# DanielQ-51/cudapathtracer

Measured on AMD Instinct MI355X. Metric: Mray/s, higher is better.
Workload: dtype f32; 1 GPU; cornell_1920x1080_1024spp_depth8_mis; spp=1024, max_depth=8, integrator=UNIDIRECTIONAL (MIS), variant=megakernel, seed=103033, triangles=36, bvh_nodes=31

## Files before the change

cudapathtracer_amd/csrc/pt_device.h:

```cpp
#pragma once
#include <hip/hip_runtime.h>
#include <stdint.h>

#define PT_DEV __device__ __forceinline__

namespace pt {

constexpr float kEps = 0.00001f;
constexpr float kRayEps = 0.001f;
constexpr float kPi = 3.141592f;

struct V3 { float x, y, z; };

PT_DEV V3 v3(float x, float y, float z) { return V3{x, y, z}; }
PT_DEV V3 v3(float a) { return V3{a, a, a}; }
PT_DEV V3 operator+(V3 a, V3 b) { return V3{a.x + b.x, a.y + b.y, a.z + b.z}; }
PT_DEV V3 operator-(V3 a, V3 b) { return V3{a.x - b.x, a.y - b.y, a.z - b.z}; }
PT_DEV V3 operator*(V3 a, float t) { return V3{a.x * t, a.y * t, a.z * t}; }
PT_DEV V3 operator*(float t, V3 a) { return V3{a.x * t, a.y * t, a.z * t}; }
PT_DEV V3 operator*(V3 a, V3 b) { return V3{a.x * b.x, a.y * b.y, a.z * b.z}; }
PT_DEV V3 operator/(V3 a, float t) { return V3{a.x / t, a.y / t, a.z / t}; }
PT_DEV V3 operator/(V3 a, V3 b) { return V3{a.x / b.x, a.y / b.y, a.z / b.z}; }
PT_DEV V3 operator-(V3 a) { return V3{-a.x, -a.y, -a.z}; }

PT_DEV float dot(V3 a, V3 b) { return __builtin_fmaf(a.z, b.z, __builtin_fmaf(a.y, b.y, a.x * b.x)); }
PT_DEV V3 cross(V3 a, V3 b) {
    return V3{__builtin_fmaf(a.y, b.z, -(a.z * b.y)), __builtin_fmaf(a.z, b.x, -(a.x * b.z)), __builtin_fmaf(a.x, b.y, -(a.y * b.x))};
}
PT_DEV float fminf_(float a, float b) { return __builtin_fminf(a, b); }
PT_DEV float fmaxf_(float a, float b) { return __builtin_fmaxf(a, b); }
#ifndef PT_FAST_RCP
#define PT_FAST_RCP 1
#endif
#ifndef PT_RCP_UNIFORM
#define PT_RCP_UNIFORM 1
#endif
PT_DEV float rcp_exact(float a) {
#if PT_FAST_RCP && PT_RCP_UNIFORM
    const float m = __builtin_fabsf(a);
    const float r0 = __builtin_amdgcn_rcpf(a);
    float r = __builtin_fmaf(r0, __builtin_fmaf(-a, r0, 1.0f), r0);
    const bool inRange = m >= 1e-12f && m <= 1.0e30f;
    if (__builtin_expect(__builtin_amdgcn_ballot_w64(!inRange) != 0ull, 0)) r = inRange ? r : 1.0f / a;
    return r;
#else
#if PT_FAST_RCP
    const float m = __builtin_fabsf(a);
    if (m >= 1e-12f && m <= 1.0e30f) {
        const float r0 = __builtin_amdgcn_rcpf(a);
        return __builtin_fmaf(r0, __builtin_fmaf(-a, r0, 1.0f), r0);
    }
#endif
    return 1.0f / a;
#endif
}
PT_DEV float rsqrt_(float x) { return rcp_exact(__builtin_sqrtf(x)); }
PT_DEV V3 normalize(V3 v) { float il = rsqrt_(dot(v, v)); return V3{v.x * il, v.y * il, v.z * il}; }
PT_DEV float length(V3 v) { return __builtin_sqrtf(dot(v, v)); }
PT_DEV float clampf(float x, float lo, float hi) { return x < lo ? lo : (x > hi ? hi : x); }

PT_DEV void sincos_(float x, float& s, float& c) {
    float k = __builtin_rintf(x * 0.636619772f);
    float r = __builtin_fmaf(k, -1.5703125f, x);
    r = __builtin_fmaf(k, -4.837512969970703125e-4f, r);
    r = __builtin_fmaf(k, -7.54978995489188216e-8f, r);
    int q = (int)k;
    float r2 = r * r;
    float ps = __builtin_fmaf(r2, -1.9515295891e-4f, 8.3321608736e-3f);
    ps = __builtin_fmaf(ps, r2, -1.6666654611e-1f);
    float sn = __builtin_fmaf(r * r2, ps, r);
    float pc = __builtin_fmaf(r2, 2.443315711809948e-5f, -1.388731625493765e-3f);
    pc = __builtin_fmaf(pc, r2, 4.166664568298827e-2f);
    float cs = __builtin_fmaf(r2 * r2, pc, __builtin_fmaf(r2, -0.5f, 1.0f));
    bool swap = q & 1;
    float a = swap ? cs : sn, b = swap ? sn : cs;
    s = (q & 2) ? -a : a;
    c = ((q + 1) & 2) ? -b : b;
}

PT_DEV float exp_(float x) {
    if (x != x) return x;
    if (x > 88.5f) return __builtin_inff();
    if (x < -87.0f) return 0.0f;
    float n = __builtin_rintf(x * 1.44269504f);
    float r = __builtin_fmaf(n, -0.693359375f, x);
    r = __builtin_fmaf(n, 2.12194440e-4f, r);
    float p = __builtin_fmaf(r, 1.9875691500e-4f, 1.3981999507e-3f);
    p = __builtin_fmaf(p, r, 8.3334519073e-3f);
// ... 108 lines not shown
```

cudapathtracer_amd/csrc/pt_megakernel.h:

```cpp
#pragma once
#include "pt_path.h"
#include "pt_params.h"

namespace pt {

PT_DEV void wave_add_total(unsigned long long* totals, int k, uint32_t v) {
    unsigned long long s = v;
    for (int off = 32; off > 0; off >>= 1) s += __shfl_down(s, off, 64);
    if ((threadIdx.x & 63) == 0 && s) atomicAdd(&totals[k], s);
}

extern __shared__ __attribute__((aligned(16))) unsigned char pt_smem[];

PT_DEV SceneCache stage_scene_cache(const DeviceScene& S, int cacheNodes, int cacheTris, int attrOff = 0, int nA = 0, int nM = 0, int nL = 0) {
    typedef __attribute__((address_space(3))) f4v lds_f4;
    lds_f4* dstN = (lds_f4*)pt_smem;
    lds_f4* dstT = dstN + cacheNodes * 4;
    const f4v* srcN = reinterpret_cast<const f4v*>(S.nodes);
    const f4v* srcT = reinterpret_cast<const f4v*>(S.tris);
    for (int i = threadIdx.x; i < cacheNodes * 4; i += blockDim.x) dstN[i] = srcN[i];
    for (int i = threadIdx.x; i < cacheTris * 3; i += blockDim.x) dstT[i] = srcT[i];
    if (attrOff > 0) {
        lds_f4* dA = (lds_f4*)(pt_smem + attrOff);
        lds_f4* dM = dA + nA * 5;
// ... 62 lines not shown
                    } else if (tmo == 0ull || now - t0 > 4ull * tmo) {
                        atomicOr((unsigned*)&q[3], 2u);
                        break;
                    }
                }
            }
            __builtin_amdgcn_s_sleep(64);
        }
    }
    return __builtin_amdgcn_readfirstlane(item);
}
PT_DEV void queue_push(int* q, int mask, int item, int lane) {
    if (lane == 0) {
        const unsigned pos = atomicAdd((unsigned*)&q[1], 1u);
        unsigned long long* slot = queue_slot(q, mask, pos);
        const unsigned long long t0 = wall_clock64();
        while ((unsigned)PT_QLOAD(slot) != pos) {
            if ((PT_QLOAD(&q[3]) & 6) != 0) return;
            if (wall_clock64() - t0 > queue_timeout(q)) { atomicOr((unsigned*)&q[3], 4u); return; }
            __builtin_amdgcn_s_sleep(4);
        }
        PT_QSTORE(slot, ((unsigned long long)(unsigned)item << 32) | (unsigned long long)(pos + 1u));
    }
}
PT_DEV uint32_t state_load(const uint32_t* p, bool shared) { return shared ? PT_QLOAD(p) : *p; }
PT_DEV void state_store(uint32_t* p, uint32_t v, bool shared) { if (shared) PT_QSTORE(p, v); else *p = v; }

template <int INTEG, bool COUNT, bool DEFER, bool ONCHIP, int STACKN, bool CULL = false, bool REFILL = false, bool FLAT = false, bool SIMPLE = false, int FLATW = 1, int TREE = 0, bool LEAN = false,
          bool MOMENTS = false>
PT_DEV void megakernel_body(const KParams& P, const MomentsK& M = MomentsK{nullptr, nullptr, 0, 0.0f}) {
    static_assert(!MOMENTS || !COUNT, "the fused moments render has no counting form");
    constexpr bool NOLEAF = SIMPLE || LEAN || (DEFER && FLAT);
    constexpr bool LTRI = DEFER && FLAT && SIMPLE;
#ifndef PT_TRISEL_SIMPLE4
#define PT_TRISEL_SIMPLE4 1
#endif
    constexpr bool TRISEL = ((PT_TRISEL_LEAN != 0 && LEAN && !SIMPLE) || (PT_TRISEL_SIMPLE4 != 0 && SIMPLE && STACKN == kStackLds)) && !ONCHIP && !COUNT;
    const int wave = threadIdx.x >> 6, lane = threadIdx.x & 63, nW = blockDim.x >> 6;
    DeviceScene S = P.S;
    constexpr bool ATTRLDS = ONCHIP && kAttrCacheBytes > 0;
    constexpr int kMedBytes = SIMPLE ? 0 : kMediumMax * 64;
    const int attrOff = ATTRLDS ? P.cacheNodes * 64 + P.cacheTris * 48 + nW * (STACKN * 256 + kMedBytes) : 0;
    DeviceScene Sstage = S;
#ifdef PT_EXPERIMENTAL
    constexpr bool WIDE = TREE == 1, COMPACT = TREE == 2;
    if (WIDE) Sstage.nodes = reinterpret_cast<const PNode*>(P.wnodes);
    if (COMPACT) Sstage.nodes = reinterpret_cast<const PNode*>(P.qnodes);
#else
    static_assert(TREE == 0, "the wide / compact trees are -DPT_EXPERIMENTAL builds (pt_trace_experimental.h)");
#endif
    const SceneCache SC = stage_scene_cache(Sstage, P.cacheNodes, P.cacheTris, attrOff, P.cacheAttrs, P.cacheMats, P.cacheLights);
    if constexpr (ATTRLDS) {
        typedef __attribute__((address_space(3))) const PAttr lds_attr;
        typedef __attribute__((address_space(3))) const PMat lds_mat;
        typedef __attribute__((address_space(3))) const PLight lds_light;
        lds_attr* a = (lds_attr*)(pt_smem + attrOff);
        lds_mat* m = (lds_mat*)(pt_smem + attrOff + P.cacheAttrs * 80);
        lds_light* l = (lds_light*)(pt_smem + attrOff + P.cacheAttrs * 80 + P.cacheMats * 96);
        S.attrs = (const PAttr*)a; S.mats = (const PMat*)m; S.lights = (const PLight*)l;
    }
    int vb = blockIdx.x;
#ifdef PT_EXPERIMENTAL
    if (P.xcdBands) {
        const int nB = gridDim.x, q = nB >> 3, r = nB & 7, x = vb & 7;
        vb = x * q + (x < r ? x : r) + (vb >> 3);
    }
// ... 176 lines not shown
                const Compact K{P.qnodes, reinterpret_cast<const f4v*>(P.leafBox), P.mids};
                trace_resume_q<STACKN>(S, SC, K, st, rs, ps.o, ps.d, (nBusy * P.refillKeep) >> 4, thr, h, Keep{P.nodeKeep, P.triKeep});
                PT_STAMP(1);
                continue;
            }
            if constexpr (WIDE) {
                trace_resume_w4<STACKN>(S, SC, P.wnodes, st, rs, ps.o, ps.d, (nBusy * P.refillKeep) >> 4, thr, h, c, Keep{P.nodeKeep, P.triKeep});
                if (!(rs.flags & kRayBusy) && (rs.flags & kRayTie)) {
                    SceneCache none; none.nodes = nullptr; none.nNodes = 0; none.tris = nullptr; none.nTris = 0;
                    trace_closest_plain<false, STACKN, false, false>(S, none, ps.o, ps.d, 999999.0f, st, h, c);
                    rs.flags &= ~kRayTie;
                }
                PT_STAMP(1);
                continue;
            }
#endif
#if !defined(PT_EXPERIMENTAL)
            trace_resume<COUNT, STACKN, ONCHIP, NOLEAF, TRISEL>(S, SC, st, rs, ps.o, ps.d, (nBusy * P.refillKeep) >> 4, thr, h, c, Keep{P.nodeKeep, P.triKeep});
#elif PT_SPEC == 2
            if (P.spec) trace_resume_spec<COUNT, STACKN, ONCHIP, NOLEAF>(S, SC, st, rs, ps.o, ps.d, (nBusy * P.refillKeep) >> 4, thr, h, c, Keep{P.nodeKeep, P.triKeep}, P.spec == 2);
            else trace_resume<COUNT, STACKN, ONCHIP, NOLEAF, TRISEL>(S, SC, st, rs, ps.o, ps.d, (nBusy * P.refillKeep) >> 4, thr, h, c, Keep{P.nodeKeep, P.triKeep});
#elif PT_SPEC == 1
            trace_resume_spec<COUNT, STACKN, ONCHIP, NOLEAF>(S, SC, st, rs, ps.o, ps.d, (nBusy * P.refillKeep) >> 4, thr, h, c, Keep{P.nodeKeep, P.triKeep}, P.spec == 2);
#else
            trace_resume<COUNT, STACKN, ONCHIP, NOLEAF, TRISEL>(S, SC, st, rs, ps.o, ps.d, (nBusy * P.refillKeep) >> 4, thr, h, c, Keep{P.nodeKeep, P.triKeep});
#endif
            PT_STAMP(1);
            continue;
        }
#ifdef PT_STAMPS
        occ[0] += 64; occ[1] += __builtin_popcountll(__ballot((ps.flags & kInPath) != 0 || (samplesLeft > 0 && !stopStarting)));
#endif
        const uint32_t flagsIn = ps.flags;
        if (DEFER) apply_pending<NOLEAF>(ps, thr, acc);
        if constexpr (MOMENTS && DEFER) landed_by_apply(flagsIn);
        if (ps.flags & kInPath) {
            bool done = path_bounce<INTEG, COUNT, DEFER, SIMPLE, LEAN, NOLEAF, LTRI>(S, ps, ms, h, P.maxDepth, P.useMIS, shadowSync, c, LTRI ? P.lightTri8 : 0ull);
            if (!done) done = path_exhausted<INTEG>(ps, P.maxDepth);
            if (done) { path_finish(ps, acc, DEFER); if constexpr (MOMENTS) landed_by_finish(); }
        }
        PT_STAMP(2);
        while (!(ps.flags & kInPath) && samplesLeft > 0 && !stopStarting) {
            samplesLeft--;
            path_begin<COUNT>(P.cam, ps, ms, PT_PX, PT_PY, c);
            if (path_exhausted<INTEG>(ps, P.maxDepth)) { path_finish(ps, acc, DEFER); if constexpr (MOMENTS) landed_by_finish(); }
        }
        const bool hasExt = (ps.flags & kInPath) != 0;
        const bool hasShadow = DEFER && (ps.flags & kShadowPending) != 0;
        PT_STAMP(0);
#ifdef PT_STAMPS
        occ[2] += __builtin_popcountll(__ballot(hasExt)); occ[3] += __builtin_popcountll(__ballot(hasShadow));
#endif
        if (__ballot(hasExt || hasShadow) == 0ull) break;
        if constexpr (DEFER && FLAT) {
            trace_pair_flat<STACKN>(S, SC, st, hasShadow, ps.so, ps.sd, ps.smaxt, LTRI ? (ps.flags & kLightTriMask) >> kLightTriShift : 0u, hasExt, ps.o, ps.d, thr, h, c, P.cacheNodes, P.leaves, P.nLeaves);
#ifdef PT_DIAG_DOUBLE_PAIR
            { Hit h2; V3 thr2; trace_pair_flat<STACKN>(S, SC, st, hasShadow, ps.so, ps.sd, ps.smaxt, LTRI ? (ps.flags & kLightTriMask) >> kLightTriShift : 0u, hasExt, ps.o, ps.d, thr2, h2, c, P.cacheNodes, P.leaves, P.nLeaves);
              if (hasExt && h2.tri == h.tri) h.t = fminf_(h.t, h2.t); thr.x = fminf_(thr.x, thr2.x); }
#endif
        }
#ifdef PT_EXPERIMENTAL
        else if (DEFER) trace_pair<COUNT, STACKN>(S, SC, st, hasShadow, ps.so, ps.sd, ps.smaxt, hasExt, ps.o, ps.d, thr, h, c);
#endif
        else if constexpr (FLAT) {
            trace_closest_flat<STACKN, FLATW>(S, SC, hasExt, ps.o, ps.d, 999999.0f, st, h, c, P.cacheNodes, P.leaves, P.nLeaves);
#ifdef PT_DIAG_DOUBLE_CLOSEST
            { Hit h2; trace_closest_flat<STACKN, FLATW>(S, SC, hasExt, ps.o, ps.d, 999999.0f, st, h2, c, P.cacheNodes); if (hasExt && h2.tri == h.tri) h.t = fminf_(h.t, h2.t); }
#endif
        }
        else if (hasExt) trace_closest<COUNT, STACKN, ONCHIP, CULL>(S, SC, ps.o, ps.d, 999999.0f, st, h, c, Keep{P.nodeKeep, P.triKeep});
        PT_STAMP(1);
    }

    if (lpt) {
        if (lane == 0) { atomicAdd(&P.queue[4], -myRem); atomicAdd(&P.queue[5], -1); }
        __builtin_amdgcn_s_setprio(0);
    }
#ifdef PT_STAMPS
    if (P.totals && lane == 0) {
        for (int k = 0; k < 3; k++) atomicAdd(&P.totals[8 + k], stamp[k]);
        atomicAdd(&P.totals[14], stamp[3]);
        const unsigned long long wall1 = wall_clock64();
        atomicAdd(&P.totals[11], wall1 - wall0);
        atomicMax(&P.totals[12], ~wall0);
        atomicMax(&P.totals[13], wall1);
        if (!COUNT) {
            atomicAdd(&P.totals[0], occ[2]); atomicAdd(&P.totals[1], occ[3]);
            atomicAdd(&P.totals[7], occ[1]); atomicAdd(&P.totals[15], occ[0]);
        }
    }
// ... 119 lines not shown
```

cudapathtracer_amd/csrc/pt_path.h:

```cpp
#pragma once
#include "pt_shade.h"

namespace pt {

struct HitInfo { V3 point, normal, emission; float uvx, uvy, dist; int tri, material, lightInd; bool backface; };

PT_DEV void resolve_hit(const DeviceScene& S, const Hit& h, V3 o, V3 d, HitInfo& hi) {
    const PAttr& at = S.attrs[h.tri];
    float bz = 1.0f - h.u - h.v;
    hi.point = v3(__builtin_fmaf(h.t, d.x, o.x), __builtin_fmaf(h.t, d.y, o.y), __builtin_fmaf(h.t, d.z, o.z));
    V3 n = normalize(ld3(at.n0) * bz + ld3(at.n1) * h.u + ld3(at.n2) * h.v);
    hi.uvx = at.uv0[0] * bz + at.uv1[0] * h.u + at.uv2[0] * h.v;
    hi.uvy = at.uv0[1] * bz + at.uv1[1] * h.u + at.uv2[1] * h.v;
    if (dot(n, d) > 0.0f) { n = -n; hi.backface = true; } else hi.backface = false;
    hi.normal = n;
    hi.material = at.material;
    hi.emission = ld3(at.emission);
    hi.lightInd = at.lightInd;
    hi.tri = h.tri;
    hi.dist = h.t;
}

enum : uint32_t {
    kInPath = 1u,
    kHitFirstNonSpec = 2u,
    kShadowPending = 4u,
    kNeeValid = 8u,
    kFinishPending = 16u,
    kLightTriShift = 8u, kLightTriMask = 0x7fu << 8,
};

struct PathState {
    Rng rng;
    V3 o, d;
    V3 beta, Li, prevPoint, woLocal;
    float pdf, etaI, etaT;
    int depth, guard, msTop;
    uint32_t flags;
    V3 so, sd; float smaxt;
    V3 neeRaw, neeBeta; float neeW;
};

struct LdsMedium {
    typedef __attribute__((address_space(3))) uint8_t lds_u8;
    lds_u8* p;
    PT_DEV int get(int i) const { return p[i * 64]; }
    PT_DEV void set(int i, int v) { p[i * 64] = (uint8_t)v; }
};
struct NoMedium {
    PT_DEV int get(int) const { return 0; }
    PT_DEV void set(int, int) {}
};
struct RegMedium {
    uint32_t w0, w1, w2, w3;
    PT_DEV int get(int i) const {
        uint32_t w = (i < 8) ? ((i < 4) ? w0 : w1) : ((i < 12) ? w2 : w3);
        return (int)((w >> ((i & 3) * 8)) & 0xffu);
    }
    PT_DEV void set(int i, int v) {
        uint32_t sh = (uint32_t)(i & 3) * 8u, m = ~(0xffu << sh), b = ((uint32_t)v & 0xffu) << sh;
        if (i < 4) w0 = (w0 & m) | b; else if (i < 8) w1 = (w1 & m) | b; else if (i < 12) w2 = (w2 & m) | b; else w3 = (w3 & m) | b;
    }
};

template <class MS>
PT_DEV void medium_remove(MS& ms, int& top, int materialID) {
    int found = -1;
    for (int i = top - 1; i > 0; i--) if (ms.get(i) == materialID) { found = i; break; }
    if (found != -1) {
        for (int i = found; i < top - 1; i++) ms.set(i, ms.get(i + 1));
        top--;
    }
}

template <bool COUNT, class MS>
PT_DEV void path_begin(const CamK& cam, PathState& ps, MS& ms, int x, int y, Ctr& c) {
    camera_ray<COUNT>(cam, ps.rng, x, y, ps.o, ps.d, c);
    const bool fin = (ps.flags & kFinishPending) != 0;
    ps.beta = v3(1.0f); ps.Li = v3(fin ? ps.Li.x : 0.0f, fin ? ps.Li.y : 0.0f, fin ? ps.Li.z : 0.0f); ps.prevPoint = v3(0.0f); ps.woLocal = v3(0.0f);
    ps.pdf = kEps; ps.etaI = kEps; ps.etaT = kEps;
    ps.depth = 0; ps.guard = 0; ps.msTop = 1; ms.set(0, 0);
    ps.flags = (ps.flags & ~kHitFirstNonSpec) | kInPath;
}

template <bool PRE = false>
PT_DEV void apply_pending(PathState& ps, V3 thr, V3& acc) {
    const bool fin = (ps.flags & kFinishPending) != 0;
    const bool add = (ps.flags & kShadowPending) && (ps.flags & kNeeValid) && dot(thr, thr) > 0.0f;
    V3 term = ps.neeRaw;
    if (!PRE) term = (ps.neeBeta * (ps.neeRaw * thr)) * ps.neeW;
    const V3 sum = ps.Li + term;
    const V3 li = v3(add ? sum.x : ps.Li.x, add ? sum.y : ps.Li.y, add ? sum.z : ps.Li.z);
    const V3 done = acc + li;
    acc = v3(fin ? done.x : acc.x, fin ? done.y : acc.y, fin ? done.z : acc.z);
    ps.Li = v3(fin ? 0.0f : li.x, fin ? 0.0f : li.y, fin ? 0.0f : li.z);
    ps.flags &= ~(kShadowPending | kNeeValid | kFinishPending | kLightTriMask);
}

template <int INTEG>
PT_DEV bool path_exhausted(PathState& ps, int maxDepth) {
    if (ps.depth >= ((INTEG == 2) ? maxDepth : 100)) return true;
    if (INTEG != 2 && ++ps.guard > 4096) return true;
    return false;
}

struct NeeRecord { V3 so, sd; float smaxt; V3 neeRaw, neeBeta; float neeW; };

template <int INTEG, bool COUNT, bool DEFER, bool SIMPLE, bool LEAN, bool PRE, bool LTRI, class MS, class ShadowFn>
PT_DEV bool bounce_core(const DeviceScene& S, Rng& rng, V3& o, V3& d, V3& beta, V3& Li, V3& prevPoint, V3& woLocal,
                        float& pdf, float& etaI, float& etaT, int& depth, int& msTop, uint32_t& flags, NeeRecord& nr,
                        MS& ms, const Hit& h, int maxDepth, int useMIS, ShadowFn shadow, Ctr& c, uint64_t lightTri8) {
    if (COUNT) c.iters++;
    if (h.tri < 0) {
        Li = Li + beta * v3(0.0f);
        return true;
    }
    HitInfo hi;
    resolve_hit(S, h, o, d, hi);
    const PMat& m = S.mats[hi.material];
    if (INTEG == 2) {
        const Onb frame = onb_of(hi.normal);
        V3 toSurface = to_local(d, frame);
        V3 f = v3(0.0f), toNext = v3(0.0f);
        float p = 0.0f;
        if (SIMPLE) cosine_sample_f<COUNT>(rng, ld3(m.albedo), toNext, f, p, c, m.albedoOverPi);
        else sample_f_eval<COUNT, LEAN>(rng, m, S.textures, toSurface, 1.0f, hi.backface, toNext, f, p, hi.uvx, hi.uvy, c);
        if (p <= 0.0f || dot(f, f) < kEps) return true;
        Li = Li + hi.emission * beta;
        beta = beta * ((f * __builtin_fabsf(toNext.z)) / p);
        V3 nw = to_world(toNext, frame);
        o = hi.point + ((toNext.z > 0.0f) ? (hi.normal * kRayEps) : ((-hi.normal) * kRayEps));
        d = nw;
        depth++;
        return false;
    }
    const Onb frame = onb_of(hi.normal);
    V3 wiLocal = to_local(d, frame);
    bool isSpecular = false, trueHit = true;
    if (!SIMPLE) {
        isSpecular = (m.flags & kMatSpecular) != 0;
        int minPriorID = ms.get(0);
        int minPrior = S.mats[minPriorID].priority;
        for (int i = 1; i < msTop; i++) {
            int id = ms.get(i);
            int pr = S.mats[id].priority;
            if (pr < minPrior) { minPrior = pr; minPriorID = id; }
        }
        const PMat& dom = S.mats[minPriorID];
        if (hi.dist > kEps && !(dom.absorption[0] == 0.0f && dom.absorption[1] == 0.0f && dom.absorption[2] == 0.0f)) {
            V3 att = v3(exp_(-dom.absorption[0] * hi.dist), exp_(-dom.absorption[1] * hi.dist), exp_(-dom.absorption[2] * hi.dist));
            beta = beta * att;
        }
        if (m.flags & kMatBoundary) {
            if (m.priority <= minPrior) {
                if (m.type == 2) {
                    etaI = dom.ior;
                    if (!hi.backface) etaT = m.ior;
                    else if (msTop == 1) etaT = 1.0f;
                    else {
                        int mp = 99, second = ms.get(0);
                        for (int i = 0; i < msTop; i++) {
                            int id = ms.get(i);
                            int pr = S.mats[id].priority;
                            if (pr) { if (mp > pr && id != hi.material) { second = id; mp = pr; } }
                        }
                        etaT = S.mats[second].ior;
                    }
                }
            } else {
                trueHit = false;
                if (!hi.backface) { if (msTop < 16) { ms.set(msTop, hi.material); msTop++; } }
                else medium_remove(ms, msTop, hi.material);
            }
        } else etaI = dom.ior;
    }
    bool done = false;
    if (trueHit) {
        float le2 = dot(hi.emission, hi.emission);
        if (le2 > kEps) {
            if (depth == 0 || !(flags & kHitFirstNonSpec)) Li = Li + beta * hi.emission;
            else if (useMIS && !isSpecular) {
                float lightPdf = kEps;
                if (hi.lightInd >= 0) {
                    const PLight& L = S.lights[hi.lightInd];
                    V3 s2l = hi.point - prevPoint;
                    V3 wi = normalize(s2l);
                    float dist2 = dot(s2l, s2l);
                    float cosL = dot(ld3(L.na), -wi);
                    lightPdf = dist2 / (cosL * (float)S.nLights * L.area);
                }
                if (lightPdf > kEps) {
                    float wB = pdf * pdf / (lightPdf * lightPdf + pdf * pdf);
                    Li = Li + (beta * hi.emission) * wB;
                }
            }
        }
        if (useMIS && le2 < kEps && !isSpecular && S.nLights > 0) {
            int index = min((int)(draw<COUNT>(rng, c) * (float)S.nLights), S.nLights - 1);
            const PLight& L = S.lights[index];
            if (LTRI) flags |= index < 8 ? ((uint32_t)(lightTri8 >> (uint32_t)(index * 8)) & 0x7fu) << kLightTriShift : 0u;
            V3 A = ld3(L.a), B = ld3(L.b), Cc = ld3(L.c);
            float u = __builtin_sqrtf(draw<COUNT>(rng, c));
            float v = draw<COUNT>(rng, c);
            V3 p = (1.0f - u) * A + (u * (1.0f - v)) * B + (u * v) * Cc;
            V3 s2l = p - hi.point;
            V3 wi = normalize(s2l);
            V3 ro = hi.point + wi * kEps;
            float t = length(s2l) - kEps;
            {
                float tt, uu, vv;
                if ((PT_RCP_UNIFORM ? moller_trumbore_sel : moller_trumbore)(A, B - A, Cc - A, ro, wi, tt, uu, vv)) t = tt;
// ... 1 lines not shown
            const float maxt = t * (1.0f - kEps);
            V3 thr = v3(1.0f);
            if (!DEFER) thr = shadow(ro, wi, maxt);
            if (DEFER || dot(thr, thr) > 0.0f) {
                float dist2 = dot(s2l, s2l);
                float cosL = dot(ld3(L.na), -wi);
                float cosS = __builtin_fabsf(dot(hi.normal, wi));
                float lightPdf = dist2 / (cosL * (float)S.nLights * L.area);
                V3 wiL = to_local(wi, frame);
                if (!DEFER) woLocal = wiL;
                V3 f = SIMPLE ? ld3(m.albedoOverPi) : f_eval<LEAN>(m, S.textures, wiLocal, wiL, etaI, hi.uvx, hi.uvy);
                V3 nee = ((f * ld3(L.emission)) * cosS) / lightPdf;
                if (lightPdf > kEps) {
                    float pdfB = pdf;
                    if (SIMPLE) pdfB = cosine_pdf(wiL);
                    else pdf_eval<LEAN>(m, S.textures, wiLocal, wiL, etaI, hi.uvx, hi.uvy, pdfB);
                    float wN = lightPdf * lightPdf / (pdfB * pdfB + lightPdf * lightPdf);
                    if (DEFER) {
                        if (PRE) nr.neeRaw = (beta * nee) * wN;
                        else { nr.neeRaw = nee; nr.neeBeta = beta; nr.neeW = wN; }
                        flags |= COUNT ? kNeeValid : (kNeeValid | kShadowPending);
                    } else {
                        pdf = pdfB;
                        nee = nee * thr;
                        Li = Li + (beta * nee) * wN;
                    }
                }
                if (DEFER) {
                    nr.so = ro; nr.sd = wi; nr.smaxt = maxt;
                    if (COUNT) flags |= kShadowPending;
                }
            }
        }
        V3 f = v3(0.0f);
        if (SIMPLE) cosine_sample_f<COUNT>(rng, ld3(m.albedo), woLocal, f, pdf, c, m.albedoOverPi);
        else sample_f_eval<COUNT, LEAN>(rng, m, S.textures, wiLocal, etaI, hi.backface, woLocal, f, pdf, hi.uvx, hi.uvy, c);
        V3 woWorld = to_world(woLocal, frame);
        pdf = fmaxf_(pdf, 0.01f);
        if (!SIMPLE && woLocal.z < 0.0f) {
            if (!hi.backface) { if (msTop < 16) { ms.set(msTop, hi.material); msTop++; } }
            else medium_remove(ms, msTop, hi.material);
        }
        beta = beta * ((f * __builtin_fabsf(woLocal.z)) / pdf);
        if (woLocal.z > 0.0f) o = hi.point + hi.normal * kEps;
        else o = hi.point - hi.normal * kEps;
        d = normalize(woWorld);
        prevPoint = hi.point;
    } else {
        woLocal = wiLocal;
        o = hi.point + d * kRayEps;
        depth--;
    }
    if (depth > maxDepth) {
        float lum = dot(beta, v3(0.2126f, 0.7152f, 0.0722f));
        float p = clampf(lum, 0.05f, 0.99f);
        if (draw<COUNT>(rng, c) > p) done = true;
        else beta = beta / p;
    }
    if (!done) {
        if (!isSpecular) flags |= kHitFirstNonSpec;
        depth++;
    }
    return done;
}


template <int INTEG, bool COUNT, bool DEFER, bool SIMPLE = false, bool LEAN = false, bool PRE = SIMPLE, bool LTRI = false, class MS, class ShadowFn>
PT_DEV bool path_bounce(const DeviceScene& S, PathState& ps, MS& ms, const Hit& h, int maxDepth, int useMIS, ShadowFn shadow, Ctr& c, uint64_t lightTri8 = 0ull) {
    Rng rng = ps.rng;
    V3 o = ps.o, d = ps.d, beta = ps.beta, Li = ps.Li, prevPoint = ps.prevPoint, woLocal = ps.woLocal;
    float pdf = ps.pdf, etaI = ps.etaI, etaT = ps.etaT;
    int depth = ps.depth, msTop = ps.msTop;
    uint32_t flags = ps.flags;
    NeeRecord nr;
#ifndef PT_NR_FRESH
#define PT_NR_FRESH 1
#endif
#if PT_NR_FRESH
    nr.so = v3(0.0f); nr.sd = v3(0.0f); nr.smaxt = 0.0f; nr.neeRaw = v3(0.0f); nr.neeBeta = v3(0.0f); nr.neeW = 0.0f;
#else
    nr.so = ps.so; nr.sd = ps.sd; nr.smaxt = ps.smaxt; nr.neeRaw = ps.neeRaw; nr.neeBeta = ps.neeBeta; nr.neeW = ps.neeW;
#endif
    bool done = bounce_core<INTEG, COUNT, DEFER, SIMPLE, LEAN, PRE, LTRI>(S, rng, o, d, beta, Li, prevPoint, woLocal, pdf, etaI, etaT, depth, msTop, flags, nr,
                                                 ms, h, maxDepth, useMIS, shadow, c, lightTri8);
    ps.rng = rng;
    ps.o = o; ps.d = d; ps.beta = beta; ps.Li = Li; ps.prevPoint = prevPoint; ps.woLocal = woLocal;
    ps.pdf = pdf; ps.etaI = etaI; ps.etaT = etaT; ps.depth = depth; ps.msTop = msTop; ps.flags = flags;
    ps.so = nr.so; ps.sd = nr.sd; ps.smaxt = nr.smaxt; ps.neeRaw = nr.neeRaw; ps.neeBeta = nr.neeBeta; ps.neeW = nr.neeW;
    return done;
}

}
```

cudapathtracer_amd/csrc/pt_shade.h:

```cpp
#pragma once
#include "pt_trace.h"

namespace pt {

template <bool COUNT>
PT_DEV float draw(Rng& r, Ctr& c) { if (COUNT) c.draws++; return rng_uniform(r); }

template <bool COUNT>
PT_DEV void camera_ray(const CamK& cam, Rng& rng, int x, int y, V3& o, V3& d, Ctr& c) {
    float aspect = (float)cam.w / (float)cam.h;
    float jitterX = (draw<COUNT>(rng, c) - 0.5f) * cam.jitter;
    float jitterY = (draw<COUNT>(rng, c) - 0.5f) * cam.jitter;
    float u = (2.0f * (((float)x + jitterX) / (float)cam.w) - 1.0f) * aspect * cam.fovScale;
    float v = (2.0f * (((float)y + jitterY) / (float)cam.h) - 1.0f) * cam.fovScale;
    V3 focal = cam.origin + (cam.right * (u * cam.focalDist)) + (cam.up * (v * cam.focalDist)) + (cam.forward * cam.focalDist);
    V3 lens = v3(0.0f);
    if (cam.aperture > 0.0f) {
        float r_rnd = draw<COUNT>(rng, c);
        float theta = 2.0f * 3.141592f * draw<COUNT>(rng, c);
        float radius = cam.aperture * __builtin_sqrtf(r_rnd);
        float sn, cs; sincos_(theta, sn, cs);
        lens = (cam.right * (radius * cs)) + (cam.up * (radius * sn));
    }
    o = cam.origin + lens;
    d = normalize(focal - o);
}

PT_DEV V3 onb_tangent(V3 n) {
    if (__builtin_fabsf(n.x) > __builtin_fabsf(n.z)) return normalize(v3(-n.y, n.x, 0.0f));
    return normalize(v3(0.0f, -n.z, n.y));
}
PT_DEV V3 to_world(V3 l, V3 n) {
    V3 t = onb_tangent(n);
    V3 b = cross(n, t);
    return l.x * t + l.y * b + l.z * n;
}
PT_DEV V3 to_local(V3 w, V3 n) {
    V3 t = onb_tangent(n);
    V3 b = cross(n, t);
    return v3(dot(w, t), dot(w, b), dot(w, n));
}
struct Onb { V3 t, b, n; };
PT_DEV Onb onb_of(V3 n) { Onb f; f.t = onb_tangent(n); f.b = cross(n, f.t); f.n = n; return f; }
PT_DEV V3 to_world(V3 l, const Onb& f) { return l.x * f.t + l.y * f.b + l.z * f.n; }
PT_DEV V3 to_local(V3 w, const Onb& f) { return v3(dot(w, f.t), dot(w, f.b), dot(w, f.n)); }

PT_DEV V3 cosine_f(V3 base) { return base / kPi; }
PT_DEV float cosine_pdf(V3 wo) { return fmaxf_(wo.z, kEps) / kPi; }

template <bool COUNT>
PT_DEV void cosine_sample_f(Rng& rng, V3 base, V3& wo, V3& f, float& pdf, Ctr& c, const float* fPre = nullptr) {
    float u1 = draw<COUNT>(rng, c);
    u1 = fminf_(u1, 1.0f - kEps);
    float u2 = draw<COUNT>(rng, c);
    float r = __builtin_sqrtf(u1);
    float phi = 2.0f * kPi * u2;
    float sn, cs; sincos_(phi, sn, cs);
    wo = v3(r * cs, r * sn, __builtin_sqrtf(1.0f - u1));
    f = fPre ? ld3(fPre) : cosine_f(base);
    pdf = cosine_pdf(wo);
}

PT_DEV float D_GGX(V3 h, float alpha) {
    float c = h.z;
    float a2 = alpha * alpha;
    float denom = c * c * (a2 - 1.0f) + 1.0f;
    return a2 / (kPi * denom * denom);
}
PT_DEV float G1_GGX(V3 v, float alpha) {
    float c = v.z;
    float tanTheta = __builtin_sqrtf(1.0f - c * c) / c;
    float a = 1.0f / (alpha * tanTheta);
    if (a < 1.6f) return (3.535f * a + 2.181f * a * a) / (1.0f + 2.276f * a + 2.577f * a * a);
    return 1.0f;
}
PT_DEV float G_Smith(V3 wi, V3 wo, float alpha) { return G1_GGX(wi, alpha) * G1_GGX(wo, alpha); }
// ... 196 lines not shown
```

cudapathtracer_amd/csrc/pt_trace.h:

```cpp
#pragma once
#include "pt_device.h"

namespace pt {

struct Ctr {
    uint32_t raysClosest, raysShadow, pops, boxes, tris, hits, draws, iters;
    uint32_t gnodes;
    uint32_t gnodeFrom;
#ifdef PT_UTIL
    uint32_t u[8];
#endif
};
#ifdef PT_UTIL
#define PT_UTIL_STEP(c, k) do { if (COUNT) { (c).u[(k) + 1]++; const uint64_t e_ = __builtin_amdgcn_ballot_w64(true); \
    if (__builtin_amdgcn_mbcnt_hi((uint32_t)(e_ >> 32), __builtin_amdgcn_mbcnt_lo((uint32_t)e_, 0u)) == 0u) (c).u[k]++; } } while (0)
#else
#define PT_UTIL_STEP(c, k) do {} while (0)
#endif

typedef float f4v __attribute__((ext_vector_type(4)));
PT_DEV int32_t f2i(float f) { return __builtin_bit_cast(int32_t, f); }
PT_DEV uint32_t f2u(float f) { return __builtin_bit_cast(uint32_t, f); }
typedef __attribute__((address_space(3))) int32_t lds_i32;
typedef __attribute__((address_space(3))) const f4v lds_cf4;
// ... 5 lines not shown

template <int N>
struct Stack {
    lds_i32* lds;
    int32_t* spill;
    int sp;
    template <bool ONCHIP = false>
    PT_DEV void push(int32_t v) {
        if (ONCHIP || sp < N) lds[sp * 64] = v; else spill[(sp - N) * 64] = v;
        sp++;
    }
    template <bool ONCHIP = false>
    PT_DEV int32_t pop() {
        sp--;
        int32_t v;
        if (ONCHIP || sp < N) v = lds[sp * 64]; else v = spill[(sp - N) * 64];
        return v;
    }
};

struct Hit { float t, u, v; int32_t tri; int32_t material; };

PT_DEV V3 inv3(V3 d) {
#if PT_FAST_RCP
    const float lo = fminf_(fminf_(__builtin_fabsf(d.x), __builtin_fabsf(d.y)), __builtin_fabsf(d.z));
    const float hi = fmaxf_(fmaxf_(__builtin_fabsf(d.x), __builtin_fabsf(d.y)), __builtin_fabsf(d.z));
    if (lo >= 1e-12f && hi <= 1.0e30f) {
        const float rx = __builtin_amdgcn_rcpf(d.x), ry = __builtin_amdgcn_rcpf(d.y), rz = __builtin_amdgcn_rcpf(d.z);
        return v3(__builtin_fmaf(rx, __builtin_fmaf(-d.x, rx, 1.0f), rx), __builtin_fmaf(ry, __builtin_fmaf(-d.y, ry, 1.0f), ry),
                  __builtin_fmaf(rz, __builtin_fmaf(-d.z, rz, 1.0f), rz));
    }
#endif
    return v3(1.0f / d.x, 1.0f / d.y, 1.0f / d.z);
}

PT_DEV bool slab(float mnx, float mny, float mnz, float mxx, float mxy, float mxz, V3 o, V3 inv, float& tmin) {
    float tx1 = (mnx - o.x) * inv.x, tx2 = (mxx - o.x) * inv.x;
    float tmn = fmaxf_(-1e30f, fminf_(tx1, tx2));
    float tmx = fminf_(1e30f, fmaxf_(tx1, tx2));
    float ty1 = (mny - o.y) * inv.y, ty2 = (mxy - o.y) * inv.y;
    tmn = fmaxf_(tmn, fminf_(ty1, ty2));
    tmx = fminf_(tmx, fmaxf_(ty1, ty2));
    float tz1 = (mnz - o.z) * inv.z, tz2 = (mxz - o.z) * inv.z;
    tmn = fmaxf_(tmn, fminf_(tz1, tz2));
    tmx = fminf_(tmx, fmaxf_(tz1, tz2));
    tmin = tmn;
    return (tmx >= tmn) && (tmx > 0.0f);
}

PT_DEV bool slab_hit(float mnx, float mny, float mnz, float mxx, float mxy, float mxz, V3 o, V3 inv) {
    float tx1 = (mnx - o.x) * inv.x, tx2 = (mxx - o.x) * inv.x;
    float tmn = fmaxf_(1.401298464e-45f, fminf_(tx1, tx2));
    float tmx = fminf_(1e30f, fmaxf_(tx1, tx2));
    float ty1 = (mny - o.y) * inv.y, ty2 = (mxy - o.y) * inv.y;
    tmn = fmaxf_(tmn, fminf_(ty1, ty2));
    tmx = fminf_(tmx, fmaxf_(ty1, ty2));
    float tz1 = (mnz - o.z) * inv.z, tz2 = (mxz - o.z) * inv.z;
    tmn = fmaxf_(tmn, fminf_(tz1, tz2));
    tmx = fminf_(tmx, fmaxf_(tz1, tz2));
    return tmx >= tmn;
}

PT_DEV bool moller_trumbore(V3 v0, V3 e1, V3 e2, V3 o, V3 d, float& t, float& u, float& v) {
    V3 h = cross(d, e2);
    float a = dot(h, e1);
    if (__builtin_fabsf(a) < 1e-12f) return false;
// ... 528 lines not shown
                int32_t ref = S.rootRef;
                int lo = 0;
                while (ref >= 0) {
                    const NodeData nd = load_node<true>(S, C, ref);
                    const int mid = lo + f2i(nd.d.z), hi = mid + f2i(nd.d.w);
                    const Set inL = tied & Set::range(lo, mid - lo), inR = tied & Set::range(mid, hi - mid);
                    bool goLeft = !inR.any();
                    if (inL.any() && inR.any()) {
                        float tL, tR;
                        slab(nd.a.x, nd.a.y, nd.a.z, nd.a.w, nd.b.x, nd.b.y, o, inv, tL);
                        slab(nd.b.z, nd.b.w, nd.c.x, nd.c.y, nd.c.z, nd.c.w, o, inv, tR);
                        goLeft = tL < tR;
                    }
                    ref = goLeft ? f2i(nd.d.x) : f2i(nd.d.y);
                    if (!goLeft) lo = mid;
                    tied = goLeft ? inL : inR;
                }
                win = tied.first();
            }
            const TriData q = load_tri<true>(S, C, win);
            float t, u, v;
            moller_trumbore(v3(q.a.x, q.a.y, q.a.z), v3(q.a.w, q.b.x, q.b.y), v3(q.b.z, q.b.w, q.e.x), o, d, t, u, v);
            hit.t = t; hit.u = u; hit.v = v;
            hit.tri = (int32_t)(f2u(q.e.y) & 0x7fffffffu);
            hit.material = f2i(q.e.z);
        }
    }
    wave_lds_sync();
}

#ifndef PT_PAIR_MIN_ALWAYS
#define PT_PAIR_MIN_ALWAYS 0
#endif
template <int N>
PT_DEV void trace_pair_flat(const DeviceScene& S, const SceneCache& C, Stack<N>& st, bool hasShadow, V3 so, V3 sd, float smaxt, uint32_t ltri1,
                            bool hasExt, V3 eo, V3 ed, V3& thr, Hit& hit, Ctr& c, int nInternal, const PLeaf* __restrict__ leaves = nullptr, int nLeaves = 0) {
    static_assert(N >= 24, "the scratch layout needs 24 x 64 words of the wave's stack area");
    typedef __attribute__((address_space(3))) unsigned long long lds_u64;
    const int lane = (int)(threadIdx.x & 63u);
    lds_i32* Wd = st.lds - lane;
    typedef __attribute__((address_space(3))) f4v lds_f4;
    constexpr int kMax = 8 * 128, kKeyA = 9 * 128, kKeyB = kKeyA + 256, kPre = kKeyA;
    lds_f4* Rec = (lds_f4*)Wd;
    const V3 invE = inv3(ed), invS = inv3(sd);
    uint64_t tmE = 0ull, tmS = 0ull;
    if (S.rootRef < 0) { const uint64_t all = ~0ull >> (64 - S.nTris); tmE = hasExt ? all : 0ull; tmS = hasShadow ? all : 0ull; }
    else if (nLeaves > 0 && __builtin_amdgcn_ballot_w64((hasExt && !inv_is_regular(invE)) || (hasShadow && !inv_is_regular(invS))) == 0ull) {
        _Pragma("unroll 2")
        for (int k = 0; k < nLeaves; ++k) {
            const LeafBox L = leaf_box(leaves, k);
            const bool eH = slab_hit(L.mnx, L.mny, L.mnz, L.mxx, L.mxy, L.mxz, eo, invE);
            const bool sH = slab_hit(L.mnx, L.mny, L.mnz, L.mxx, L.mxy, L.mxz, so, invS);
            const uint64_t m = ((1ull << (uint32_t)L.count) - 1ull) << (uint32_t)L.first;
            tmE |= eH ? m : 0ull; tmS |= sH ? m : 0ull;
        }
        tmE = hasExt ? tmE : 0ull; tmS = hasShadow ? tmS : 0ull;
    } else {
        uint64_t visE = hasExt ? 1ull << (uint32_t)S.rootRef : 0ull, visS = hasShadow ? 1ull << (uint32_t)S.rootRef : 0ull;
        for (int i = 0; i < nInternal; ++i) {
            const bool vE = ((visE >> i) & 1ull) != 0ull, vS = ((visS >> i) & 1ull) != 0ull;
            if (__builtin_amdgcn_ballot_w64(vE || vS) == 0ull) continue;
            const NodeData n = load_node<true>(S, C, i);
            float t0, t1;
            const bool eL = slab(n.a.x, n.a.y, n.a.z, n.a.w, n.b.x, n.b.y, eo, invE, t0) && vE;
            const bool eR = slab(n.b.z, n.b.w, n.c.x, n.c.y, n.c.z, n.c.w, eo, invE, t1) && vE;
            const bool sL = slab(n.a.x, n.a.y, n.a.z, n.a.w, n.b.x, n.b.y, so, invS, t0) && vS;
            const bool sR = slab(n.b.z, n.b.w, n.c.x, n.c.y, n.c.z, n.c.w, so, invS, t1) && vS;
            const int32_t left = __builtin_amdgcn_readfirstlane(f2i(n.d.x)), right = __builtin_amdgcn_readfirstlane(f2i(n.d.y));
            const int32_t cntL = __builtin_amdgcn_readfirstlane(f2i(n.d.z)), cntR = __builtin_amdgcn_readfirstlane(f2i(n.d.w));
            const uint64_t bL = left >= 0 ? 1ull << (uint32_t)left : (~0ull >> (64 - cntL)) << (uint32_t)(~left);
            const uint64_t bR = right >= 0 ? 1ull << (uint32_t)right : (~0ull >> (64 - cntR)) << (uint32_t)(~right);
            if (left >= 0) { visE |= eL ? bL : 0ull; visS |= sL ? bL : 0ull; } else { tmE |= eL ? bL : 0ull; tmS |= sL ? bL : 0ull; }
            if (right >= 0) { visE |= eR ? bR : 0ull; visS |= sR ? bR : 0ull; } else { tmE |= eR ? bR : 0ull; tmS |= sR ? bR : 0ull; }
        }
    }
    tmS &= ~((1ull << ltri1) >> 1);
    auto scan = [&](int v, int& total) {
// ... 364 lines not shown
```

Measured before the change: 30330 Mray/s.

## Add branch-free arms for inv3, ONB, MIS, deferred normalize, dead-branch origin

Adds a compile-time PT_LOGIC_ARMS mask with four arms on by default for the deferred flat SIMPLE/LEAN kernels. Reciprocals are computed with a wave-uniform fallback and the ONB tangent is built from selects. The MIS emission and NEE branches are merged into one shared light-evaluation block. Direction normalization is deferred through a kDirRaw flag so it happens once before tracing. The aim is to cut divergence and duplicated math in the shading step, at the cost of more complex control flow and small numerical differences.

```diff
diff --git a/cudapathtracer_amd/csrc/pt_device.h b/cudapathtracer_amd/csrc/pt_device.h
--- a/cudapathtracer_amd/csrc/pt_device.h
+++ b/cudapathtracer_amd/csrc/pt_device.h
@@ -54,6 +54,11 @@
     return 1.0f / a;
 #endif
 }
+#ifndef PT_LOGIC_ARMS
+#define PT_LOGIC_ARMS 15
+#endif
+constexpr bool kArmInv3 = (PT_LOGIC_ARMS & 1) != 0, kArmOnb = (PT_LOGIC_ARMS & 2) != 0, kArmMis = (PT_LOGIC_ARMS & 4) != 0,
+               kArmNorm = (PT_LOGIC_ARMS & 8) != 0, kArmDead = (PT_LOGIC_ARMS & 16) != 0;
 PT_DEV float rsqrt_(float x) { return rcp_exact(__builtin_sqrtf(x)); }
 PT_DEV V3 normalize(V3 v) { float il = rsqrt_(dot(v, v)); return V3{v.x * il, v.y * il, v.z * il}; }
 PT_DEV float length(V3 v) { return __builtin_sqrtf(dot(v, v)); }
diff --git a/cudapathtracer_amd/csrc/pt_megakernel.h b/cudapathtracer_amd/csrc/pt_megakernel.h
--- a/cudapathtracer_amd/csrc/pt_megakernel.h
+++ b/cudapathtracer_amd/csrc/pt_megakernel.h
@@ -118,6 +118,7 @@
     static_assert(!MOMENTS || !COUNT, "the fused moments render has no counting form");
     constexpr bool NOLEAF = SIMPLE || LEAN || (DEFER && FLAT);
     constexpr bool LTRI = DEFER && FLAT && SIMPLE;
+    constexpr bool ARMS = DEFER && FLAT && (SIMPLE || LEAN);
 #ifndef PT_TRISEL_SIMPLE4
 #define PT_TRISEL_SIMPLE4 1
 #endif
@@ -360,19 +361,20 @@
         occ[0] += 64; occ[1] += __builtin_popcountll(__ballot((ps.flags & kInPath) != 0 || (samplesLeft > 0 && !stopStarting)));
 #endif
         const uint32_t flagsIn = ps.flags;
-        if (DEFER) apply_pending<NOLEAF>(ps, thr, acc);
+        if (DEFER) apply_pending<NOLEAF, ARMS && kArmNorm>(ps, thr, acc);
         if constexpr (MOMENTS && DEFER) landed_by_apply(flagsIn);
         if (ps.flags & kInPath) {
-            bool done = path_bounce<INTEG, COUNT, DEFER, SIMPLE, LEAN, NOLEAF, LTRI>(S, ps, ms, h, P.maxDepth, P.useMIS, shadowSync, c, LTRI ? P.lightTri8 : 0ull);
+            bool done = path_bounce<INTEG, COUNT, DEFER, SIMPLE, LEAN, NOLEAF, LTRI, ARMS>(S, ps, ms, h, P.maxDepth, P.useMIS, shadowSync, c, LTRI ? P.lightTri8 : 0ull);
             if (!done) done = path_exhausted<INTEG>(ps, P.maxDepth);
             if (done) { path_finish(ps, acc, DEFER); if constexpr (MOMENTS) landed_by_finish(); }
         }
         PT_STAMP(2);
         while (!(ps.flags & kInPath) && samplesLeft > 0 && !stopStarting) {
             samplesLeft--;
-            path_begin<COUNT>(P.cam, ps, ms, PT_PX, PT_PY, c);
+            path_begin<COUNT, ARMS && kArmNorm>(P.cam, ps, ms, PT_PX, PT_PY, c);
             if (path_exhausted<INTEG>(ps, P.maxDepth)) { path_finish(ps, acc, DEFER); if constexpr (MOMENTS) landed_by_finish(); }
         }
+        if constexpr (ARMS && kArmNorm) { if (ps.flags & kDirRaw) ps.d = normalize(ps.d); }
         const bool hasExt = (ps.flags & kInPath) != 0;
         const bool hasShadow = DEFER && (ps.flags & kShadowPending) != 0;
         PT_STAMP(0);
@@ -381,9 +383,9 @@
 #endif
         if (__ballot(hasExt || hasShadow) == 0ull) break;
         if constexpr (DEFER && FLAT) {
-            trace_pair_flat<STACKN>(S, SC, st, hasShadow, ps.so, ps.sd, ps.smaxt, LTRI ? (ps.flags & kLightTriMask) >> kLightTriShift : 0u, hasExt, ps.o, ps.d, thr, h, c, P.cacheNodes, P.leaves, P.nLeaves);
+            trace_pair_flat<STACKN, ARMS>(S, SC, st, hasShadow, ps.so, ps.sd, ps.smaxt, LTRI ? (ps.flags & kLightTriMask) >> kLightTriShift : 0u, hasExt, ps.o, ps.d, thr, h, c, P.cacheNodes, P.leaves, P.nLeaves);
 #ifdef PT_DIAG_DOUBLE_PAIR
-            { Hit h2; V3 thr2; trace_pair_flat<STACKN>(S, SC, st, hasShadow, ps.so, ps.sd, ps.smaxt, LTRI ? (ps.flags & kLightTriMask) >> kLightTriShift : 0u, hasExt, ps.o, ps.d, thr2, h2, c, P.cacheNodes, P.leaves, P.nLeaves);
+            { Hit h2; V3 thr2; trace_pair_flat<STACKN, ARMS>(S, SC, st, hasShadow, ps.so, ps.sd, ps.smaxt, LTRI ? (ps.flags & kLightTriMask) >> kLightTriShift : 0u, hasExt, ps.o, ps.d, thr2, h2, c, P.cacheNodes, P.leaves, P.nLeaves);
               if (hasExt && h2.tri == h.tri) h.t = fminf_(h.t, h2.t); thr.x = fminf_(thr.x, thr2.x); }
 #endif
         }
diff --git a/cudapathtracer_amd/csrc/pt_path.h b/cudapathtracer_amd/csrc/pt_path.h
--- a/cudapathtracer_amd/csrc/pt_path.h
+++ b/cudapathtracer_amd/csrc/pt_path.h
@@ -27,6 +27,7 @@
     kShadowPending = 4u,
     kNeeValid = 8u,
     kFinishPending = 16u,
+    kDirRaw = 32u,
     kLightTriShift = 8u, kLightTriMask = 0x7fu << 8,
 };
 
@@ -73,17 +74,17 @@
     }
 }
 
-template <bool COUNT, class MS>
+template <bool COUNT, bool RAW = false, class MS>
 PT_DEV void path_begin(const CamK& cam, PathState& ps, MS& ms, int x, int y, Ctr& c) {
-    camera_ray<COUNT>(cam, ps.rng, x, y, ps.o, ps.d, c);
+    camera_ray<COUNT, RAW>(cam, ps.rng, x, y, ps.o, ps.d, c);
     const bool fin = (ps.flags & kFinishPending) != 0;
     ps.beta = v3(1.0f); ps.Li = v3(fin ? ps.Li.x : 0.0f, fin ? ps.Li.y : 0.0f, fin ? ps.Li.z : 0.0f); ps.prevPoint = v3(0.0f); ps.woLocal = v3(0.0f);
     ps.pdf = kEps; ps.etaI = kEps; ps.etaT = kEps;
     ps.depth = 0; ps.guard = 0; ps.msTop = 1; ms.set(0, 0);
-    ps.flags = (ps.flags & ~kHitFirstNonSpec) | kInPath;
-}
-
-template <bool PRE = false>
+    ps.flags = (ps.flags & ~kHitFirstNonSpec) | (RAW ? kInPath | kDirRaw : kInPath);
+}
+
+template <bool PRE = false, bool ARMS = false>
 PT_DEV void apply_pending(PathState& ps, V3 thr, V3& acc) {
     const bool fin = (ps.flags & kFinishPending) != 0;
     const bool add = (ps.flags & kShadowPending) && (ps.flags & kNeeValid) && dot(thr, thr) > 0.0f;
@@ -94,7 +95,7 @@
     const V3 done = acc + li;
     acc = v3(fin ? done.x : acc.x, fin ? done.y : acc.y, fin ? done.z : acc.z);
     ps.Li = v3(fin ? 0.0f : li.x, fin ? 0.0f : li.y, fin ? 0.0f : li.z);
-    ps.flags &= ~(kShadowPending | kNeeValid | kFinishPending | kLightTriMask);
+    ps.flags &= ~(kShadowPending | kNeeValid | kFinishPending | kLightTriMask | (ARMS ? kDirRaw : 0u));
 }
 
 template <int INTEG>
@@ -106,10 +107,11 @@
 
 struct NeeRecord { V3 so, sd; float smaxt; V3 neeRaw, neeBeta; float neeW; };
 
-template <int INTEG, bool COUNT, bool DEFER, bool SIMPLE, bool LEAN, bool PRE, bool LTRI, class MS, class ShadowFn>
+template <int INTEG, bool COUNT, bool DEFER, bool SIMPLE, bool LEAN, bool PRE, bool LTRI, bool ARMS, class MS, class ShadowFn>
 PT_DEV bool bounce_core(const DeviceScene& S, Rng& rng, V3& o, V3& d, V3& beta, V3& Li, V3& prevPoint, V3& woLocal,
                         float& pdf, float& etaI, float& etaT, int& depth, int& msTop, uint32_t& flags, NeeRecord& nr,
                         MS& ms, const Hit& h, int maxDepth, int useMIS, ShadowFn shadow, Ctr& c, uint64_t lightTri8) {
+    static_assert(!ARMS || (DEFER && INTEG != 2 && !COUNT), "ARMS is a form of the DEFER logic step of the timed MIS kernels");
     if (COUNT) c.iters++;
     if (h.tri < 0) {
         Li = Li + beta * v3(0.0f);
@@ -134,7 +136,7 @@
         depth++;
         return false;
     }
-    const Onb frame = onb_of(hi.normal);
+    const Onb frame = onb_of<ARMS && kArmOnb>(hi.normal);
     V3 wiLocal = to_local(d, frame);
     bool isSpecular = false, trueHit = true;
     if (!SIMPLE) {
@@ -177,6 +179,64 @@
     bool done = false;
     if (trueHit) {
         float le2 = dot(hi.emission, hi.emission);
+        if constexpr (ARMS && kArmMis) {
+            const bool firstSeen = depth == 0 || !(flags & kHitFirstNonSpec);
+            const bool emArm = le2 > kEps && !firstSeen && useMIS && !isSpecular && hi.lightInd >= 0;
+            const bool neeArm = useMIS && le2 < kEps && !isSpecular && S.nLights > 0;
+            if (le2 > kEps && firstSeen) Li = Li + beta * hi.emission;
+            int li = 0;
+            V3 s2l = v3(0.0f), A = v3(0.0f), B = v3(0.0f), Cc = v3(0.0f);
+            if (neeArm) {
+                li = min((int)(draw<COUNT>(rng, c) * (float)S.nLights), S.nLights - 1);
+                const PLight& L = S.lights[li];
+                if (LTRI) flags |= li < 8 ? ((uint32_t)(lightTri8 >> (uint32_t)(li * 8)) & 0x7fu) << kLightTriShift : 0u;
+                A = ld3(L.a); B = ld3(L.b); Cc = ld3(L.c);
+                float u = __builtin_sqrtf(draw<COUNT>(rng, c));
+                float v = draw<COUNT>(rng, c);
+                V3 p = (1.0f - u) * A + (u * (1.0f - v)) * B + (u * v) * Cc;
+                s2l = p - hi.point;
+            } else if (emArm) {
+                li = hi.lightInd;
+                s2l = hi.point - prevPoint;
+            }
+            if (neeArm || emArm) {
+                const PLight& L = S.lights[li];
+                V3 wi = normalize(s2l);
+                float dist2 = dot(s2l, s2l);
+                float cosL = dot(ld3(L.na), -wi);
+                float lightPdf = dist2 / (cosL * (float)S.nLights * L.area);
+                float a = pdf, b = lightPdf;
+                V3 nee = v3(0.0f);
+                if (neeArm) {
+                    V3 ro = hi.point + wi * kEps;
+                    float t = length(s2l) - kEps;
+                    {
+                        float tt, uu, vv;
+                        if ((PT_RCP_UNIFORM ? moller_trumbore_sel : moller_trumbore)(A, B - A, Cc - A, ro, wi, tt, uu, vv)) t = tt;
+                    }
+                    const float maxt = t * (1.0f - kEps);
+                    float cosS = __builtin_fabsf(dot(hi.normal, wi));
+                    V3 wiL = to_local(wi, frame);
+                    V3 f = SIMPLE ? ld3(m.albedoOverPi) : f_eval<LEAN>(m, S.textures, wiLocal, wiL, etaI, hi.uvx, hi.uvy);
+                    nee = ((f * ld3(L.emission)) * cosS) / lightPdf;
+                    if (lightPdf > kEps) {
+                        float pdfB = pdf;
+                        if (SIMPLE) pdfB = cosine_pdf(wiL);
+                        else pdf_eval<LEAN>(m, S.textures, wiLocal, wiL, etaI, hi.uvx, hi.uvy, pdfB);
+                        a = lightPdf; b = pdfB;
+                    }
+                    nr.so = ro; nr.sd = wi; nr.smaxt = maxt;
+                }
+                if (lightPdf > kEps) {
+                    const float w = a * a / (b * b + a * a);
+                    if (neeArm) {
+                        if (PRE) nr.neeRaw = (beta * nee) * w;
+                        else { nr.neeRaw = nee; nr.neeBeta = beta; nr.neeW = w; }
+                        flags |= kNeeValid | kShadowPending;
+                    } else Li = Li + (beta * hi.emission) * w;
+                }
+            }
+        } else {
         if (le2 > kEps) {
             if (depth == 0 || !(flags & kHitFirstNonSpec)) Li = Li + beta * hi.emission;
             else if (useMIS && !isSpecular) {
@@ -244,6 +304,7 @@
                 }
             }
         }
+        }
         V3 f = v3(0.0f);
         if (SIMPLE) cosine_sample_f<COUNT>(rng, ld3(m.albedo), woLocal, f, pdf, c, m.albedoOverPi);
         else sample_f_eval<COUNT, LEAN>(rng, m, S.textures, wiLocal, etaI, hi.backface, woLocal, f, pdf, hi.uvx, hi.uvy, c);
@@ -254,9 +315,10 @@
             else medium_remove(ms, msTop, hi.material);
         }
         beta = beta * ((f * __builtin_fabsf(woLocal.z)) / pdf);
-        if (woLocal.z > 0.0f) o = hi.point + hi.normal * kEps;
+        if ((ARMS && kArmDead && SIMPLE) || woLocal.z > 0.0f) o = hi.point + hi.normal * kEps;
         else o = hi.point - hi.normal * kEps;
-        d = normalize(woWorld);
+        if constexpr (ARMS && kArmNorm) { d = woWorld; flags |= kDirRaw; }
+        else d = normalize(woWorld);
         prevPoint = hi.point;
     } else {
         woLocal = wiLocal;
@@ -277,7 +339,7 @@
 }
 
 
-template <int INTEG, bool COUNT, bool DEFER, bool SIMPLE = false, bool LEAN = false, bool PRE = SIMPLE, bool LTRI = false, class MS, class ShadowFn>
+template <int INTEG, bool COUNT, bool DEFER, bool SIMPLE = false, bool LEAN = false, bool PRE = SIMPLE, bool LTRI = false, bool ARMS = false, class MS, class ShadowFn>
 PT_DEV bool path_bounce(const DeviceScene& S, PathState& ps, MS& ms, const Hit& h, int maxDepth, int useMIS, ShadowFn shadow, Ctr& c, uint64_t lightTri8 = 0ull) {
     Rng rng = ps.rng;
     V3 o = ps.o, d = ps.d, beta = ps.beta, Li = ps.Li, prevPoint = ps.prevPoint, woLocal = ps.woLocal;
@@ -293,7 +355,7 @@
 #else
     nr.so = ps.so; nr.sd = ps.sd; nr.smaxt = ps.smaxt; nr.neeRaw = ps.neeRaw; nr.neeBeta = ps.neeBeta; nr.neeW = ps.neeW;
 #endif
-    bool done = bounce_core<INTEG, COUNT, DEFER, SIMPLE, LEAN, PRE, LTRI>(S, rng, o, d, beta, Li, prevPoint, woLocal, pdf, etaI, etaT, depth, msTop, flags, nr,
+    bool done = bounce_core<INTEG, COUNT, DEFER, SIMPLE, LEAN, PRE, LTRI, ARMS>(S, rng, o, d, beta, Li, prevPoint, woLocal, pdf, etaI, etaT, depth, msTop, flags, nr,
                                                  ms, h, maxDepth, useMIS, shadow, c, lightTri8);
     ps.rng = rng;
     ps.o = o; ps.d = d; ps.beta = beta; ps.Li = Li; ps.prevPoint = prevPoint; ps.woLocal = woLocal;
diff --git a/cudapathtracer_amd/csrc/pt_shade.h b/cudapathtracer_amd/csrc/pt_shade.h
--- a/cudapathtracer_amd/csrc/pt_shade.h
+++ b/cudapathtracer_amd/csrc/pt_shade.h
@@ -6,7 +6,7 @@
 template <bool COUNT>
 PT_DEV float draw(Rng& r, Ctr& c) { if (COUNT) c.draws++; return rng_uniform(r); }
 
-template <bool COUNT>
+template <bool COUNT, bool RAW = false>
 PT_DEV void camera_ray(const CamK& cam, Rng& rng, int x, int y, V3& o, V3& d, Ctr& c) {
     float aspect = (float)cam.w / (float)cam.h;
     float jitterX = (draw<COUNT>(rng, c) - 0.5f) * cam.jitter;
@@ -23,12 +23,19 @@
         lens = (cam.right * (radius * cs)) + (cam.up * (radius * sn));
     }
     o = cam.origin + lens;
-    d = normalize(focal - o);
+    d = RAW ? focal - o : normalize(focal - o);
 }
 
 PT_DEV V3 onb_tangent(V3 n) {
     if (__builtin_fabsf(n.x) > __builtin_fabsf(n.z)) return normalize(v3(-n.y, n.x, 0.0f));
     return normalize(v3(0.0f, -n.z, n.y));
+}
+PT_DEV V3 onb_tangent_sel(V3 n) {
+    const bool xArm = __builtin_fabsf(n.x) > __builtin_fabsf(n.z);
+    const float p = xArm ? n.x : n.y, q = xArm ? n.y : n.z;
+    const float il = rsqrt_(__builtin_fmaf(p, p, q * q));
+    const V3 v = v3(xArm ? -n.y : 0.0f, xArm ? n.x : -n.z, xArm ? 0.0f : n.y);
+    return V3{v.x * il, v.y * il, v.z * il};
 }
 PT_DEV V3 to_world(V3 l, V3 n) {
     V3 t = onb_tangent(n);
@@ -41,7 +48,8 @@
     return v3(dot(w, t), dot(w, b), dot(w, n));
 }
 struct Onb { V3 t, b, n; };
-PT_DEV Onb onb_of(V3 n) { Onb f; f.t = onb_tangent(n); f.b = cross(n, f.t); f.n = n; return f; }
+template <bool SEL = false>
+PT_DEV Onb onb_of(V3 n) { Onb f; f.t = SEL ? onb_tangent_sel(n) : onb_tangent(n); f.b = cross(n, f.t); f.n = n; return f; }
 PT_DEV V3 to_world(V3 l, const Onb& f) { return l.x * f.t + l.y * f.b + l.z * f.n; }
 PT_DEV V3 to_local(V3 w, const Onb& f) { return v3(dot(w, f.t), dot(w, f.b), dot(w, f.n)); }
 
diff --git a/cudapathtracer_amd/csrc/pt_trace.h b/cudapathtracer_amd/csrc/pt_trace.h
--- a/cudapathtracer_amd/csrc/pt_trace.h
+++ b/cudapathtracer_amd/csrc/pt_trace.h
@@ -61,6 +61,22 @@
     }
 #endif
     return v3(1.0f / d.x, 1.0f / d.y, 1.0f / d.z);
+}
+PT_DEV V3 inv3_uniform(V3 d, bool has) {
+#if PT_FAST_RCP
+    const float lo = fminf_(fminf_(__builtin_fabsf(d.x), __builtin_fabsf(d.y)), __builtin_fabsf(d.z));
+    const float hi = fmaxf_(fmaxf_(__builtin_fabsf(d.x), __builtin_fabsf(d.y)), __builtin_fabsf(d.z));
+    const float rx = __builtin_amdgcn_rcpf(d.x), ry = __builtin_amdgcn_rcpf(d.y), rz = __builtin_amdgcn_rcpf(d.z);
+    V3 r = v3(__builtin_fmaf(rx, __builtin_fmaf(-d.x, rx, 1.0f), rx), __builtin_fmaf(ry, __builtin_fmaf(-d.y, ry, 1.0f), ry),
+              __builtin_fmaf(rz, __builtin_fmaf(-d.z, rz, 1.0f), rz));
+    const bool out = has && !(lo >= 1e-12f && hi <= 1.0e30f);
+    if (__builtin_expect(__builtin_amdgcn_ballot_w64(out) != 0ull, 0)) {
+        if (out) r = v3(1.0f / d.x, 1.0f / d.y, 1.0f / d.z);
+    }
+    return r;
+#else
+    return v3(1.0f / d.x, 1.0f / d.y, 1.0f / d.z);
+#endif
 }
 
 PT_DEV bool slab(float mnx, float mny, float mnz, float mxx, float mxy, float mxz, V3 o, V3 inv, float& tmin) {
@@ -655,7 +671,7 @@
 #ifndef PT_PAIR_MIN_ALWAYS
 #define PT_PAIR_MIN_ALWAYS 0
 #endif
-template <int N>
+template <int N, bool ARMS = false>
 PT_DEV void trace_pair_flat(const DeviceScene& S, const SceneCache& C, Stack<N>& st, bool hasShadow, V3 so, V3 sd, float smaxt, uint32_t ltri1,
                             bool hasExt, V3 eo, V3 ed, V3& thr, Hit& hit, Ctr& c, int nInternal, const PLeaf* __restrict__ leaves = nullptr, int nLeaves = 0) {
     static_assert(N >= 24, "the scratch layout needs 24 x 64 words of the wave's stack area");
@@ -665,7 +681,9 @@
     typedef __attribute__((address_space(3))) f4v lds_f4;
     constexpr int kMax = 8 * 128, kKeyA = 9 * 128, kKeyB = kKeyA + 256, kPre = kKeyA;
     lds_f4* Rec = (lds_f4*)Wd;
-    const V3 invE = inv3(ed), invS = inv3(sd);
+    V3 invE, invS;
+    if constexpr (ARMS && kArmInv3) { invE = inv3_uniform(ed, hasExt); invS = inv3_uniform(sd, hasShadow); }
+    else { invE = inv3(ed); invS = inv3(sd); }
     uint64_t tmE = 0ull, tmS = 0ull;
     if (S.rootRef < 0) { const uint64_t all = ~0ull >> (64 - S.nTris); tmE = hasExt ? all : 0ull; tmS = hasShadow ? all : 0ull; }
     else if (nLeaves > 0 && __builtin_amdgcn_ballot_w64((hasExt && !inv_is_regular(invE)) || (hasShadow && !inv_is_regular(invS))) == 0ull) {
```

Measured after the change: 31230 Mray/s, median of 6. 3.0% higher.
